# sp-uhh/audio-visual-vad

Measured on AMD Instinct MI355X. Metric: AV frame-pairs/sec (fwd+bwd), higher is better.
Workload: dtype f32; 1 GPU; AV_net fused training step (WaveNet-W0 encoder + ResNet-18 trunk + concat + 2xLSTM1024 + FC, masked BCE, backward, RCCL all-reduce, fused Adam): BASELINE configs[3]/[4] per-GPU shard; per_gpu_frame_pairs=1024, global_frame_pairs=1024, sequences_per_gpu=64, parallelism=dp1, reserved_cus=0, reported_block=median

## Files before the change

### audio-visual-vad_amd/avvad/_lib.py

```python
import ctypes as C
import os

import torch

_HERE = os.path.dirname(os.path.abspath(__file__))
LIB_PATH = os.environ.get("AVVAD_LIB") or os.path.join(os.path.dirname(_HERE), "lib", "libavvad_hip.so")

TRUNK_NCONV = 20
ABI_VERSION = 3
SCORE_CHUNK = 4096
_ERR = {-1: "AVVAD_EINVAL (bad descriptor / unsupported shape)", -2: "AVVAD_EWORKSPACE (workspace too small)",
        -3: "AVVAD_ELAUNCH (kernel launch failed)"}

FP = C.c_void_p


class AvvadError(RuntimeError):
    pass


class GemmDesc(C.Structure):
    _fields_ = [(n, C.c_int) for n in ("M", "N", "K", "lda", "ldb", "ldc", "transA", "transB", "accumulate",
                                       "split_k", "relu_a", "relu_b")]

# ... 13 lines not shown
    _fields_ = [("N", C.c_int), ("H", C.c_int), ("W", C.c_int), ("training", C.c_int), ("momentum", C.c_float),
                ("eps", C.c_float), ("save_for_backward", C.c_int)]


class TrunkParams(C.Structure):
    _fields_ = [("conv_w", FP * TRUNK_NCONV), ("bn_w", FP * TRUNK_NCONV), ("bn_b", FP * TRUNK_NCONV),
                ("bn_rm", FP * TRUNK_NCONV), ("bn_rv", FP * TRUNK_NCONV)]


class TrunkGrads(C.Structure):
    _fields_ = [("conv_w", FP * TRUNK_NCONV), ("bn_w", FP * TRUNK_NCONV), ("bn_b", FP * TRUNK_NCONV)]


class ConvDesc(C.Structure):
    _fields_ = [(n, C.c_int) for n in ("N", "H", "W", "C", "Co", "KS", "stride", "pad")]


class McbDesc(C.Structure):
    _fields_ = [("rows", C.c_int), ("A", C.c_int), ("V", C.c_int), ("D", C.c_int), ("eps", C.c_float),
                ("training", C.c_int), ("momentum", C.c_float), ("save_for_backward", C.c_int)]


class StftDesc(C.Structure):
    _fields_ = [("B", C.c_int), ("L", C.c_long), ("n_fft", C.c_int), ("hop", C.c_int), ("T", C.c_int), ("eps", C.c_float)]


class StftStreamDesc(C.Structure):
    _fields_ = [("B", C.c_int), ("L", C.c_int), ("n_fft", C.c_int), ("hop", C.c_int), ("T", C.c_int), ("M", C.c_int),
                ("eps", C.c_float), ("norm_eps", C.c_float)]

# ... 25 lines not shown
    "avvad_version": (C.c_char_p, []),
    "avvad_abi_version": (C.c_int, []),
    "avvad_set_option": (C.c_int, [C.c_char_p, C.c_int]),
    "avvad_get_option": (C.c_int, [C.c_char_p]),
    "avvad_engine_workspace": (C.c_size_t, []),
    "avvad_gemm_f32": (C.c_int, [FP, FP, FP, FP, C.POINTER(GemmDesc), FP, C.c_size_t, FP]),
    "avvad_wavenet_workspace": (C.c_size_t, [C.POINTER(WavenetDesc)]),
    "avvad_wavenet_fwd": (C.c_int, [FP, C.POINTER(WavenetPtrs), FP, C.POINTER(WavenetDesc), FP, C.c_size_t, FP]),
    "avvad_wavenet_bwd": (C.c_int, [FP, C.POINTER(WavenetPtrs), FP, C.POINTER(WavenetPtrs), FP,
                                    C.POINTER(WavenetDesc), FP, C.c_size_t, FP]),
    "avvad_wavenet_block_fwd": (C.c_int, [FP, FP, FP, FP, FP, FP, C.c_int, C.c_int, C.c_int, FP]),
    "avvad_conv2d_pack_weights": (C.c_int, [FP, FP, FP, C.POINTER(ConvDesc), FP]),
    "avvad_conv2d_fwd": (C.c_int, [FP, FP, FP, C.POINTER(ConvDesc), FP, C.c_size_t, FP]),
    "avvad_conv2d_dgrad": (C.c_int, [FP, FP, FP, C.POINTER(ConvDesc), C.c_int, FP, C.c_size_t, FP]),
    "avvad_conv2d_wgrad": (C.c_int, [FP, FP, FP, C.POINTER(ConvDesc), FP, C.c_size_t, FP]),
    "avvad_conv2d_pack_weights_bf16": (C.c_int, [FP, FP, FP, C.POINTER(ConvDesc), FP]),
    "avvad_conv2d_fwd_bf16": (C.c_int, [FP, FP, FP, C.POINTER(ConvDesc), FP, C.c_size_t, FP]),
    "avvad_conv2d_dgrad_bf16": (C.c_int, [FP, FP, FP, C.POINTER(ConvDesc), C.c_int, FP, C.c_size_t, FP]),
    "avvad_conv2d_wgrad_bf16": (C.c_int, [FP, FP, FP, C.POINTER(ConvDesc), FP, C.c_size_t, FP]),
    "avvad_trunk_workspace": (C.c_size_t, [C.POINTER(TrunkDesc)]),
    "avvad_trunk_activation": (C.c_int, [C.POINTER(TrunkDesc), C.c_int, C.POINTER(C.c_size_t), C.POINTER(C.c_int), C.POINTER(C.c_int),
                                         C.POINTER(C.c_int)]),
    "avvad_trunk_fwd": (C.c_int, [FP, C.POINTER(TrunkParams), FP, C.POINTER(TrunkDesc), FP, C.c_size_t, FP]),
    "avvad_trunk_bwd": (C.c_int, [FP, C.POINTER(TrunkParams), FP, C.POINTER(TrunkGrads), C.POINTER(TrunkDesc), FP,
                                  C.c_size_t, FP]),
    "avvad_lstm_workspace": (C.c_size_t, [C.POINTER(LstmDesc)]),
    "avvad_lstm_layer_fwd": (C.c_int, [FP, FP, FP, FP, FP, FP, C.POINTER(LstmDesc), FP, C.c_size_t, FP]),
    "avvad_lstm_layer_bwd": (C.c_int, [FP, FP, FP, FP, FP, FP, FP, FP, FP, FP, C.POINTER(LstmDesc), FP, C.c_size_t, FP]),
    "avvad_lstm_state_workspace": (C.c_size_t, [C.POINTER(LstmDesc)]),
    "avvad_lstm_layer_fwd_state": (C.c_int, [FP] * 10 + [C.POINTER(LstmDesc), FP, C.c_size_t, FP]),
# ... 107 lines not shown
```

### audio-visual-vad_amd/csrc/bn_kernels.h

```cpp
#pragma once
#include "common.h"

constexpr int BN_MAXC = 1024;
constexpr int MAXC = BN_MAXC;
constexpr int STAT_CHUNKS = 512;

template <int MODE>
__global__ void __launch_bounds__(256)
    col_reduce(const float* __restrict__ x, const float* __restrict__ dy, const float* __restrict__ ymask,
               const float* __restrict__ mean, const float* __restrict__ invstd, long M, int C, long rows_per_chunk,
               double* __restrict__ part, const float* __restrict__ msc = nullptr, const float* __restrict__ msh = nullptr,
               const unsigned char* __restrict__ qmask = nullptr) {
  __shared__ double sm[256 * 8];
  const int t = threadIdx.x;
  const int Q = C >> 2, RL = 256 / Q;
  const int q = t % Q, rl = t / Q;
  double s[4] = {0, 0, 0, 0}, ss[4] = {0, 0, 0, 0};
  float mu[4] = {0, 0, 0, 0}, is[4] = {1, 1, 1, 1};
  float ksc[4] = {0, 0, 0, 0}, ksh[4] = {0, 0, 0, 0};
  if (MODE == 1) {
#pragma unroll
    for (int j = 0; j < 4; ++j) { mu[j] = mean[q * 4 + j]; is[j] = invstd[q * 4 + j]; }
    if (msc) {
#pragma unroll
// ... 158 lines not shown
    const float4 v = reinterpret_cast<const float4*>(x)[i];
    float o[4] = {bn_affine(v.x, sc.x, sh.x), bn_affine(v.y, sc.y, sh.y), bn_affine(v.z, sc.z, sh.z), bn_affine(v.w, sc.w, sh.w)};
    if (idn) {
      const float4 d = IB ? load_quad_bf16(idn, i) : reinterpret_cast<const float4*>(idn)[i];
      if (iscale) {
        o[0] += bn_affine(d.x, a.x, b.x); o[1] += bn_affine(d.y, a.y, b.y);
        o[2] += bn_affine(d.z, a.z, b.z); o[3] += bn_affine(d.w, a.w, b.w);
      } else { o[0] += d.x; o[1] += d.y; o[2] += d.z; o[3] += d.w; }
    }
    if (relu) { o[0] = fmaxf(o[0], 0.f); o[1] = fmaxf(o[1], 0.f); o[2] = fmaxf(o[2], 0.f); o[3] = fmaxf(o[3], 0.f); }
    if constexpr (OB) store_quad_bf16(y, i, o);
    else reinterpret_cast<float4*>(y)[i] = make_float4(o[0], o[1], o[2], o[3]);
    if (qmask_out)
      qmask_out[i] = (unsigned char)((o[0] > 0.f ? 1 : 0) | (o[1] > 0.f ? 2 : 0) | (o[2] > 0.f ? 4 : 0) | (o[3] > 0.f ? 8 : 0));
  }
}

template <bool OB = false>
__global__ void __launch_bounds__(256)
    bn_bwd_apply(const float* __restrict__ x, const float* dy, const float* __restrict__ ymask,
                 const float* __restrict__ mean, const float* __restrict__ invstd, const float* __restrict__ coef,
                 float* dx, float* gout, long nquad, int C, const float* __restrict__ msc = nullptr,
                 const float* __restrict__ msh = nullptr, const unsigned char* __restrict__ qmask = nullptr) {
  const bool fixed = (256 % (C >> 2)) == 0;
  long i = (long)blockIdx.x * blockDim.x + threadIdx.x;
  int c = (int)((i * 4) % C);
  float4 mu = ld4(mean, c), is = ld4(invstd, c), k0 = ld4(coef, c), k1 = ld4(coef + MAXC, c), k2 = ld4(coef + 2 * MAXC, c);
  float4 ms = make_float4(0, 0, 0, 0), mh = ms;
  if (msc) { ms = ld4(msc, c); mh = ld4(msh, c); }
  for (; i < nquad; i += (long)gridDim.x * blockDim.x) {
// ... 16 lines not shown
      if (!(qm & 1u)) g[0] = 0.f;
      if (!(qm & 2u)) g[1] = 0.f;
      if (!(qm & 4u)) g[2] = 0.f;
      if (!(qm & 8u)) g[3] = 0.f;
    } else if (msc) {
      if (!(fmaf(xv.x, ms.x, mh.x) > 0.f)) g[0] = 0.f;
      if (!(fmaf(xv.y, ms.y, mh.y) > 0.f)) g[1] = 0.f;
      if (!(fmaf(xv.z, ms.z, mh.z) > 0.f)) g[2] = 0.f;
      if (!(fmaf(xv.w, ms.w, mh.w) > 0.f)) g[3] = 0.f;
    }
    const float xs[4] = {xv.x, xv.y, xv.z, xv.w};
    const float m4[4] = {mu.x, mu.y, mu.z, mu.w}, i4[4] = {is.x, is.y, is.z, is.w};
    const float a4[4] = {k0.x, k0.y, k0.z, k0.w}, b4[4] = {k1.x, k1.y, k1.z, k1.w}, c4[4] = {k2.x, k2.y, k2.z, k2.w};
    float o[4];
#pragma unroll
    for (int j = 0; j < 4; ++j) {
      const float xh = (xs[j] - m4[j]) * i4[j];
      o[j] = a4[j] * (g[j] - b4[j] - xh * c4[j]);
    }
    if constexpr (OB) store_quad_bf16(dx, i, o);
    else reinterpret_cast<float4*>(dx)[i] = make_float4(o[0], o[1], o[2], o[3]);
    if (gout) reinterpret_cast<float4*>(gout)[i] = make_float4(g[0], g[1], g[2], g[3]);
  }
}
```

### audio-visual-vad_amd/csrc/common.h

```cpp
#pragma once
#include <hip/hip_runtime.h>
#include <stdint.h>
#include <atomic>

#include "avvad.h"

typedef float f32x16 __attribute__((ext_vector_type(16)));
typedef float f32x4 __attribute__((ext_vector_type(4)));

#include <stdio.h>
#define AVVAD_LAUNCH_CHECK()                                                                      \
  do {                                                                                            \
    hipError_t e_ = hipGetLastError();                                                            \
    if (e_ != hipSuccess) {                                                                       \
      fprintf(stderr, "avvad: HIP error '%s' after launch at %s:%d\n", hipGetErrorString(e_), __FILE__, __LINE__); \
      return AVVAD_ELAUNCH;                                                                       \
    }                                                                                             \
  } while (0)

#define AVVAD_ENTER() (void)hipGetLastError()

struct AvvadTune {
  int igemm_variant;
  int no_streamk;
// ... 6 lines not shown
  int wn_no_tail_pair;
  int wn_no_fused_wgrad;
  int no_fixup1;
  int no_buf;
  int wn_flat;
  int wn_dx;
  int wn_grid;
  int wn_bwd_t;
  int bf16;
  int stagger;
  int cls_cap;
  int no_cls;
  int no_fused_stats;
  int no_s2_cls;
  int no_conv64;
  int bwd_max_cus;
  int max_cus;
};
AvvadTune& avvad_tune();
struct BwdCuCap {
  int saved;
  BwdCuCap() : saved(avvad_tune().max_cus) {
    const int b = avvad_tune().bwd_max_cus;
    if (b > 0 && (saved <= 0 || b < saved)) avvad_tune().max_cus = b;
  }
  ~BwdCuCap() { avvad_tune().max_cus = saved; }
};

template <auto Kernel>
int allow_large_lds(size_t bytes, size_t limit) {
// ... 79 lines not shown
```

### audio-visual-vad_amd/csrc/conv64.h

```cpp
#pragma once
#include "common.h"

namespace conv64 {

constexpr int NW = 8;
constexpr int WROWS = 9 * 64;

template <bool FLIP>
__global__ void __launch_bounds__(NW * 64, 2)
    kernel(const float* __restrict__ x, const float* __restrict__ wpk, float* __restrict__ y, const int M, const int H, const int W,
           const unsigned mg_hw, const unsigned mg_w, const int accumulate, double* __restrict__ stat) {
  __shared__ __attribute__((aligned(16))) float wl[WROWS * 64 + NW * 64 * 4];
  const int t = threadIdx.x, lane = t & 63, wave = t >> 6;
  const int li = lane & 31, lh = lane >> 5;
  const __amdgpu_buffer_rsrc_t rx = brsrc2g(x);
  const __amdgpu_buffer_rsrc_t ry = brsrc2g(y);
  const long T = ((long)M + 31) / 32, G = gridDim.x;
  const long t_lo = blockIdx.x * T / G, t_hi = (blockIdx.x + 1) * T / G;
  const int HW = H * W;
  const float* const bl = wl + lh * 256 + li;

  int mbase = 0, rmask = 0, cmask = 0;
  auto tile_ctx = [&](long tile) {
    const int m = (int)tile * 32 + li;
// ... 263 lines not shown
    if (lh == 0) {
      red[(wave * 64 + li) * 2 + 0] = ds0; red[(wave * 64 + li) * 2 + 1] = dq0;
      red[(wave * 64 + li + 32) * 2 + 0] = ds1; red[(wave * 64 + li + 32) * 2 + 1] = dq1;
    }
    __syncthreads();
    if (t < 64) {
      double sa = 0, sb = 0;
#pragma unroll
      for (int w = 0; w < NW; ++w) { sa += red[(w * 64 + t) * 2 + 0]; sb += red[(w * 64 + t) * 2 + 1]; }
      stat[((long)blockIdx.x * 2 + 0) * 64 + t] = sa;
      stat[((long)blockIdx.x * 2 + 1) * 64 + t] = sb;
    }
  }
}

constexpr int WG_WAVES = 12;
constexpr int WG_MAXW = 18;
constexpr int WG_PART = WROWS * 64;

__global__ void __launch_bounds__(WG_WAVES * 64, 3)
    wgrad_kernel(const float* __restrict__ x, const float* __restrict__ dy, float* __restrict__ part, const int NR, const int H,
                 const int W, const unsigned mg_H) {
  constexpr int XP = (WG_MAXW + 2) * 64;
  constexpr int DP = (WG_MAXW + 2) * 64;
  __shared__ __attribute__((aligned(16))) float lds[2 * (3 * XP + DP)];
  const int t = threadIdx.x, lane = t & 63, wave = t >> 6;
  const int li = lane & 31, lh = lane >> 5;
  const int q = wave / 3, kh = wave - q * 3, cb = q >> 1, nb = q & 1;
  for (int i = t; i < 2 * (3 * XP + DP) / 4; i += WG_WAVES * 64) reinterpret_cast<float4*>(lds)[i] = make_float4(0.f, 0.f, 0.f, 0.f);
  const __amdgpu_buffer_rsrc_t rx = brsrc2g(x);
  const __amdgpu_buffer_rsrc_t rd = brsrc2g(dy);
  const long G = gridDim.x;
  const int r_lo = (int)(blockIdx.x * (long)NR / G), r_hi = (int)((blockIdx.x + 1) * (long)NR / G);
  const int per_row = W * 16, items = 4 * per_row;
  int sel[2], goff[2], loff[2];
#pragma unroll
  for (int u = 0; u < 2; ++u) {
    const int idx = t + u * WG_WAVES * 64;
    const int rs = idx / per_row, rem = idx - rs * per_row, px = rem >> 4, c4 = rem & 15;
    sel[u] = idx < items ? rs : -1;
    goff[u] = ((rs < 3 ? rs - 1 : 0) * W + px) * 256 + c4 * 16;
    loff[u] = rs < 3 ? rs * XP + (px + 1) * 64 + c4 * 4 : 3 * XP + px * 64 + c4 * 4;
  }
  f4v st[2];
  auto fetch = [&](int r) {
    const int n = mg_H ? (int)__umulhi((unsigned)r, mg_H) : r, h = r - n * H;
    const int rb = r * W * 256;
#pragma unroll
    for (int u = 0; u < 2; ++u) {
      const bool ok = sel[u] == 3 || (sel[u] >= 0 && (unsigned)(h + sel[u] - 1) < (unsigned)H);
      const int vo = ok ? rb + goff[u] : BUF_OOB;
      st[u] = sel[u] == 3 ? bload4(rd, vo, 0) : bload4(rx, vo, 0);
    }
  };
  auto put = [&](int buf) {
#pragma unroll
    for (int u = 0; u < 2; ++u)
      if (sel[u] >= 0) *reinterpret_cast<f4v*>(lds + buf * (3 * XP + DP) + loff[u]) = st[u];
  };
  f32x16 acc[3];
#pragma unroll
  for (int k = 0; k < 3; ++k)
#pragma unroll
    for (int r = 0; r < 16; ++r) acc[k][r] = 0.f;
  const int nks = (W + 1) >> 1;
  __syncthreads();
  if (r_lo < r_hi) {
    fetch(r_lo);
    put(0);
  }
  __syncthreads();
  for (int r = r_lo; r < r_hi; ++r) {
    const int buf = (r - r_lo) & 1;
    if (r + 1 < r_hi) fetch(r + 1);
    const float* const ap = lds + buf * (3 * XP + DP) + kh * XP + lh * 64 + cb * 32 + li;
    const float* const bp = lds + buf * (3 * XP + DP) + 3 * XP + lh * 64 + nb * 32 + li;
#pragma unroll 3
    for (int ks = 0; ks < nks; ++ks) {
      const float b = bp[ks * 128];
      const float a0 = ap[ks * 128], a1 = ap[ks * 128 + 64], a2 = ap[ks * 128 + 128];
      acc[0] = mfma32(a0, b, acc[0]);
      acc[1] = mfma32(a1, b, acc[1]);
      acc[2] = mfma32(a2, b, acc[2]);
    }
    if (r + 1 < r_hi) put(buf ^ 1);
    __syncthreads();
  }
  float* const P = part + (long)blockIdx.x * WG_PART;
#pragma unroll
  for (int kw = 0; kw < 3; ++kw)
#pragma unroll
    for (int r = 0; r < 16; ++r)
      P[((kh * 3 + kw) * 64 + cb * 32 + mfma32_row(r, lh)) * 64 + nb * 32 + li] = acc[kw][r];
}

__global__ void __launch_bounds__(256)
    wgrad_reduce(const float* __restrict__ part, const int G, float* __restrict__ out) {
  __shared__ float4 red[3][64];
  const int c = threadIdx.x & 63, gq = threadIdx.x >> 6;
  const long e4 = (long)blockIdx.x * 64 + c;
// ... 24 lines not shown
```

### audio-visual-vad_amd/csrc/misc.hip

```cpp
#include "common.h"

extern "C" const char* avvad_version(void) { return "avvad-hip 0.1 (gfx950, fp32 MFMA)"; }
extern "C" int avvad_abi_version(void) { return AVVAD_ABI_VERSION; }

#include <stdlib.h>
#include <string.h>
namespace {
struct OptName { const char* name; const char* env; int AvvadTune::*field; };
const OptName kOpts[] = {
    {"igemm_variant", "AVVAD_IGEMM_VARIANT", &AvvadTune::igemm_variant},
    {"no_streamk", "AVVAD_NO_STREAMK", &AvvadTune::no_streamk},
    {"kmajor", "AVVAD_KMAJOR", &AvvadTune::kmajor},
    {"lstm_no_fused_step", "AVVAD_LSTM_NO_FUSED_STEP", &AvvadTune::lstm_no_fused_step},
    {"lstm_no_persistent", "AVVAD_LSTM_NO_PERSISTENT", &AvvadTune::lstm_no_persistent},
    {"no_stem_kernel", "AVVAD_NO_STEM_KERNEL", &AvvadTune::no_stem_kernel},
    {"no_tall", "AVVAD_NO_TALL", &AvvadTune::no_tall},
    {"wn_no_fused_tail", "AVVAD_WN_NO_FUSED_TAIL", &AvvadTune::wn_no_fused_tail},
    {"wn_no_tail_pair", "AVVAD_WN_NO_TAIL_PAIR", &AvvadTune::wn_no_tail_pair},
    {"wn_no_fused_wgrad", "AVVAD_WN_NO_FUSED_WGRAD", &AvvadTune::wn_no_fused_wgrad},
    {"wn_bwd_t", "AVVAD_WN_BWD_T", &AvvadTune::wn_bwd_t},
    {"no_buf", "AVVAD_NO_BUF", &AvvadTune::no_buf},
    {"no_fixup1", "AVVAD_NO_FIXUP1", &AvvadTune::no_fixup1},
    {"no_conv64", "AVVAD_NO_CONV64", &AvvadTune::no_conv64},
    {"no_s2_cls", "AVVAD_NO_S2_CLS", &AvvadTune::no_s2_cls},
    {"wn_flat", "AVVAD_WN_FLAT", &AvvadTune::wn_flat},
    {"wn_grid", "AVVAD_WN_GRID", &AvvadTune::wn_grid},
    {"wn_dx", "AVVAD_WN_DX", &AvvadTune::wn_dx},
    {"bf16", "AVVAD_BF16", &AvvadTune::bf16},
    {"no_fused_stats", "AVVAD_NO_FUSED_STATS", &AvvadTune::no_fused_stats},
    {"no_cls", "AVVAD_NO_CLS", &AvvadTune::no_cls},
    {"cls_cap", "AVVAD_CLS_CAP", &AvvadTune::cls_cap},
    {"stagger", "AVVAD_STAGGER", &AvvadTune::stagger},
    {"max_cus", "AVVAD_MAX_CUS", &AvvadTune::max_cus},
    {"bwd_max_cus", "AVVAD_BWD_MAX_CUS", &AvvadTune::bwd_max_cus},
};
int parse_opt(const char* name, const char* v) {
  if (!strcmp(name, "igemm_variant")) return v[0] == 'd' ? 0 : (v[0] == 's' ? 1 : (v[0] == 'w' ? 2 : atoi(v)));
  if (!strcmp(name, "no_streamk")) return v[0] == 'a' ? 1 : (v[0] >= '0' && v[0] <= '9' && !v[1] ? 10 + (v[0] - '0') : atoi(v));
  if (!strcmp(name, "max_cus") || !strcmp(name, "bwd_max_cus") || !strcmp(name, "wn_flat") || !strcmp(name, "wn_grid") || !strcmp(name, "wn_dx") || !strcmp(name, "wn_bwd_t") || !strcmp(name, "no_fixup1") || !strcmp(name, "cls_cap")) return atoi(v);
  return (v[0] && strcmp(v, "0")) ? 1 : 0;
}
}

AvvadTune& avvad_tune() {
  static AvvadTune t = [] {
    AvvadTune x;
    memset(&x, 0, sizeof(x));
    x.igemm_variant = -1;
    for (const OptName& o : kOpts) {
      const char* v = getenv(o.env);
      if (v && v[0]) x.*(o.field) = parse_opt(o.name, v);
    }
    return x;
  }();
// ... 279 lines not shown
```

### audio-visual-vad_amd/csrc/trunk.hip

```cpp
#include "bgemm.h"
#include "conv64.h"

using convop::Geom;

namespace {

#include "bn_kernels.h"

constexpr int NCONV = AVVAD_TRUNK_NCONV;

struct ConvSpec {
  int cin, cout, ks, stride, pad;
  int stage;
  int role;
};

struct Plan {
  int N, H, W;
  int h[6], w[6];
  ConvSpec conv[NCONV];
  Geom geom[NCONV];
  size_t wf[NCONV], wd[NCONV];
  size_t wf16[NCONV], wd16[NCONV];
  size_t bn_scale, bn_shift, bn_mean, bn_invstd;
// ... 706 lines not shown
}
static inline igemm::TapSched tap_sched(const Geom& g, int tiles_per_tap) {
  const int NP = cdiv(g.N, 128) * 128;
  const int lsh = ((g.Ho - 1) * g.stride - g.pad + 2 > g.H - 1) ? 1 : 0, lsw = ((g.Wo - 1) * g.stride - g.pad + 2 > g.W - 1) ? 1 : 0;
  return igemm::TapSched{g.Ho, g.Wo, tiles_per_tap, NP / 32, 3, 1, lsh, 1, lsw};
}
static int conv_wgrad_tap(const float* x, const float* dy, float* pk, const Geom& g, hipStream_t s, float* slab) {
  const int M = 9 * g.C;
  const igemm::TapSched sc = tap_sched(g, (g.C / 128) * cdiv(g.Co, 128));
  convop::WgradXTap a{x, g, M, g.C, g.N, convop::div_magic(g.C), sc};
  convop::ColDyTap b{dy, g, g.Co, g.C, g.N, sc};
  igemm::EpiTap e{pk, g.Co, nullptr, 0};
  e.Mrows = M; e.sched = sc;
  return igemm::launch_cls(a, b, e, M, g.Co, s, slab);
}
static int conv64_wgrad(const float* x, const float* dy, float* pk, const Geom& g, hipStream_t s, float* slab) {
  const int NR = g.N * g.H;
  const int grid = NR < conv64_cus() ? NR : conv64_cus();
  hipLaunchKernelGGL(conv64::wgrad_kernel, dim3(grid), dim3(conv64::WG_WAVES * 64), 0, s, x, dy, slab, NR, g.H, g.W,
                     convop::div_magic((unsigned)g.H));
  hipLaunchKernelGGL(conv64::wgrad_reduce, dim3(conv64::WG_PART / 256), dim3(256), 0, s, (const float*)slab, grid, pk);
  AVVAD_LAUNCH_CHECK();
  return AVVAD_OK;
}
static int conv_wgrad(const float* x, const float* dy, float* pk, const Geom& g, hipStream_t s, float* slab) {
  const ConvForm f = wgrad_form(g, false, slab);
  switch (f.form) {
    case STEM: {
      const int LDW = (g.W + 6) | 1;
      const int nb = g.N < 256 ? g.N : 256;
      hipLaunchKernelGGL(stem_wgrad_mfma, dim3(nb), dim3(256), (size_t)(g.H + 6) * LDW * sizeof(float), s, x, dy, slab, g.N, g.H, g.W,
                         g.Ho, g.Wo, LDW);
      hipLaunchKernelGGL(stem_wgrad_reduce, dim3(49 * 64 / 32), dim3(256), 0, s, slab, nb, pk);
      AVVAD_LAUNCH_CHECK();
      return AVVAD_OK;
    }
    case CONV64: return conv64_wgrad(x, dy, pk, g, s, slab);
    case TAP: return conv_wgrad_tap(x, dy, pk, g, s, slab);
    default: return f.buf ? conv_wgrad_t<true>(x, dy, pk, g, f, s, slab) : conv_wgrad_t<false>(x, dy, pk, g, f, s, slab);
  }
}

static int conv_fwd16(const float* x16, const float* wf16, float* y, const Geom& g, hipStream_t s, float* slab, double* stat) {
  if (!bf16_conv_ok(g)) return AVVAD_EINVAL;
  const ConvForm f = fwd_form(g, true, slab);
  if (f.form == CONV64) return conv64_launch(true, false, x16, wf16, y, g, 0, s, stat);
  Geom gp = g;
  gp.C = g.C / 2;
  if (f.form == CLS) {
    const int MB = cdiv(g.N, 128), P = g.Ho * g.Wo;
    const igemm::ClassSched sc = fwd_sched(g, 64);
    const igemm::ClassRow cr{P, convop::div_magic(P)};
// ... 93 lines not shown
  const int C = p->conv[i].cout;
  StatCtx sc = stat_ctx(p, ws, M, C);
  if (const int n = fused_chunks(p, i, d)) {
    sc.nchunk = n;
  } else if (d->training) {
    hipLaunchKernelGGL(col_reduce<0>, dim3(sc.nchunk), dim3(256), 0, s, craw, (const float*)nullptr, (const float*)nullptr,
                       (const float*)nullptr, (const float*)nullptr, M, C, sc.rows_per_chunk, sc.part);
  }
  hipLaunchKernelGGL(bn_finalize, dim3(cdiv(C, FIN_CH)), dim3(256), 0, s, sc.part, sc.nchunk, M, C, prm->bn_w[i], prm->bn_b[i],
                     prm->bn_rm[i], prm->bn_rv[i], d->training, d->momentum, d->eps, ws + p->bn_scale + i * MAXC,
                     ws + p->bn_shift + i * MAXC, ws + p->bn_mean + i * MAXC, ws + p->bn_invstd + i * MAXC);
  AVVAD_LAUNCH_CHECK();
  return AVVAD_OK;
}

static int bn_backward(Plan* p, float* ws, int i, const float* xraw, const float* dy, const float* ymask, float* dx,
                       float* gout, long M, const avvad_trunk_params* prm, const avvad_trunk_grads* g,
                       const avvad_trunk_desc* d, hipStream_t s, bool own_relu = false, const unsigned char* qmask = nullptr,
                       bool out16 = false, int reduced_chunks = 0) {
  const int C = p->conv[i].cout;
  StatCtx sc = stat_ctx(p, ws, M, C);
  const float* mean = ws + p->bn_mean + i * MAXC;
  const float* invstd = ws + p->bn_invstd + i * MAXC;
  const float* msc = own_relu ? ws + p->bn_scale + i * MAXC : (const float*)nullptr;
  const float* msh = own_relu ? ws + p->bn_shift + i * MAXC : (const float*)nullptr;
  if (own_relu) ymask = nullptr;
  const bool qred = out16 && qmask != nullptr;
  if (reduced_chunks > 0)
    sc.nchunk = reduced_chunks;
  else
    hipLaunchKernelGGL(col_reduce<1>, dim3(sc.nchunk), dim3(256), 0, s, xraw, dy, qred ? (const float*)nullptr : ymask, mean, invstd, M, C,
                       sc.rows_per_chunk, sc.part, msc, msh, qred ? qmask : (const unsigned char*)nullptr);
  hipLaunchKernelGGL(bn_bwd_finalize, dim3(cdiv(C, FIN_CH)), dim3(256), 0, s, sc.part, sc.nchunk, M, C, prm->bn_w[i], invstd,
                     d->training, g->bn_w[i], g->bn_b[i], ws + p->coef);
  const long nq = M * C / 4;
  auto apply = out16 ? bn_bwd_apply<true> : bn_bwd_apply<false>;
  hipLaunchKernelGGL(apply, dim3(ew_grid(nq)), dim3(256), 0, s, xraw, dy, qmask ? (const float*)nullptr : ymask, mean, invstd,
                     ws + p->coef, dx, gout, nq, C, msc, msh, qmask);
  AVVAD_LAUNCH_CHECK();
  return AVVAD_OK;
}

}

static bool conv_geom(const avvad_conv_desc* d, Geom* g) {
  if (!d || d->N <= 0 || d->H <= 0 || d->W <= 0 || d->C <= 0 || d->Co <= 0 || d->KS <= 0 || d->stride <= 0 || d->pad < 0)
    return false;
  const int Ho = (d->H + 2 * d->pad - d->KS) / d->stride + 1, Wo = (d->W + 2 * d->pad - d->KS) / d->stride + 1;
  if (Ho <= 0 || Wo <= 0 || (d->stride != 1 && d->stride != 2)) return false;
// ... 40 lines not shown
#endif
extern "C" int avvad_conv2d_dgrad(const float* dy, const float* wd, float* dx, const avvad_conv_desc* d, int accumulate,
                                  void* ws, size_t ws_bytes, avvad_stream_t s) {
  AVVAD_ENTER();
  Geom g;
  if (!dy || !wd || !dx || !conv_geom(d, &g) || ws_misaligned(ws)) return AVVAD_EINVAL;
  return conv_dgrad(dy, wd, dx, g, accumulate, (hipStream_t)s, slab_of(ws, ws_bytes));
}
extern "C" int avvad_conv2d_wgrad(const float* x, const float* dy, float* dw_packed, const avvad_conv_desc* d, void* ws,
                                  size_t ws_bytes, avvad_stream_t s) {
  AVVAD_ENTER();
  Geom g;
  if (!x || !dy || !dw_packed || !conv_geom(d, &g) || ws_misaligned(ws)) return AVVAD_EINVAL;
  return conv_wgrad(x, dy, dw_packed, g, (hipStream_t)s, slab_of(ws, ws_bytes));
}

namespace {
__global__ void pack_weights_bf16(const float* __restrict__ w, __bf16* __restrict__ wf16, __bf16* __restrict__ wd16, int Co, int C, int KS) {
  const int T = KS * KS, n = Co * C * T;
  for (int i = blockIdx.x * blockDim.x + threadIdx.x; i < n; i += gridDim.x * blockDim.x) {
    int r = i;
    const int tap = r % T; r /= T;
    const int c = r % C; const int co = r / C;
    const __bf16 v = (__bf16)w[i];
    wf16[(long)co * (T * C) + ((c >> 6) * T + tap) * 64 + (c & 63)] = v;
    if (wd16) wd16[(long)c * (T * Co) + ((co >> 6) * T + tap) * 64 + (co & 63)] = v;
  }
}
}
extern "C" int avvad_conv2d_pack_weights_bf16(const float* w_oihw, void* wf16, void* wd16, const avvad_conv_desc* d, avvad_stream_t s) {
  AVVAD_ENTER();
// ... 142 lines not shown
  float* G1 = ws + p.G[1];
  float* G2 = ws + p.G[2];
  float* G3 = ws + p.G[3];
  hipLaunchKernelGGL(avgpool_bwd, dim3(ew_grid(N * p.h[5] * p.w[5] * 512)), dim3(256), 0, s, dfeat, G0, d->N,
                     p.h[5] * p.w[5], 512);
  const bool b16 = native_bf16();
  auto wgrad = [&](int i, const float* xin, const float* dyraw) -> int {
    if (!g->conv_w[i]) return AVVAD_OK;
    if (b16 && i > 0) return conv_wgrad16(xin, dyraw, ws + p.wg[i], p.geom[i], s, ws + p.slab);
    return conv_wgrad(xin, dyraw, ws + p.wg[i], p.geom[i], s, ws + p.slab);
  };
  auto dgrad = [&](const float* dyv, int i, float* dxv, int accumulate) -> int {
    if (b16) return conv_dgrad16(dyv, ws + p.wd16[i], dxv, p.geom[i], accumulate, s, ws + p.slab);
    return conv_dgrad(dyv, ws + p.wd[i], dxv, p.geom[i], accumulate, s, ws + p.slab);
  };
  int ci = NCONV;
  for (int st = 3; st >= 0; --st)
    for (int b = 1; b >= 0; --b) {
      const bool ds = (b == 0 && st > 0);
      ci -= ds ? 3 : 2;
      const int i1 = ci, i2 = ci + 1, id = ci + 2;
      const size_t* o = p.blk[st * 2 + b];
      const float* x = (st == 0 && b == 0) ? ws + p.p0 : (b == 1 ? ws + p.blk[st * 2][4] : ws + p.blk[st * 2 - 1][4]);
      const long M = N * p.h[st + 2] * p.w[st + 2];
      const unsigned char* qmb = reinterpret_cast<const unsigned char*>(ws + p.qm[st * 2 + b]);
      if (ds) {
        if ((rc = bn_backward(&p, ws, i2, ws + o[2], G0, ws + o[4], G1, nullptr, M, prm, g, d, s, false, qmb, b16))) return rc;
        if ((rc = bn_backward(&p, ws, id, ws + o[3], G0, ws + o[4], G2, nullptr, M, prm, g, d, s, false, qmb, b16))) return rc;
        if ((rc = wgrad(id, x, G2))) return rc;
        if ((rc = dgrad(G2, id, G3, 0))) return rc;
      } else {
        if ((rc = bn_backward(&p, ws, i2, ws + o[2], G0, ws + o[4], G1, G3, M, prm, g, d, s, false, qmb, b16))) return rc;
      }
      if ((rc = wgrad(i2, ws + o[1], G1))) return rc;
      if ((rc = dgrad(G1, i2, G2, 0))) return rc;
      if ((rc = bn_backward(&p, ws, i1, ws + o[0], G2, ws + o[1], G1, nullptr, M, prm, g, d, s, true, nullptr, b16))) return rc;
      if ((rc = wgrad(i1, x, G1))) return rc;
      if ((rc = dgrad(G1, i1, G3, 1))) return rc;
      float* t = G0; G0 = G3; G3 = t;
    }
  if (g->conv_w[0] || g->bn_w[0] || g->bn_b[0]) {
    float* g0 = ws + p.g0;
    const bool fuse0 = !avvad_tune().no_fused_stats;
    int grid0 = ew_grid(N * p.h[1] * p.w[1] * 16);
    if (fuse0 && grid0 > 2048) grid0 = 2048;
    hipLaunchKernelGGL(stem_pool_relu_bwd, dim3(grid0), dim3(256), 0, s, ws + p.c0,
                       ws + p.bn_scale, ws + p.bn_shift, reinterpret_cast<const unsigned*>(ws + p.am), G0, g0, d->N, p.h[1], p.w[1],
                       p.h[2], p.w[2], fuse0 ? ws + p.bn_mean : (const float*)nullptr, fuse0 ? ws + p.bn_invstd : (const float*)nullptr,
                       fuse0 ? reinterpret_cast<double*>(ws + p.part) : (double*)nullptr);
    const long M0 = N * p.h[1] * p.w[1];
    if ((rc = bn_backward(&p, ws, 0, ws + p.c0, g0, nullptr, g0, nullptr, M0, prm, g, d, s, false, nullptr, false, fuse0 ? grid0 : 0))) return rc;
    if ((rc = wgrad(0, frames, g0))) return rc;
// ... 22 lines not shown
```

### include/avvad.h

```cpp
#ifndef AVVAD_H
#define AVVAD_H

#include <stddef.h>
#include <stdint.h>

#ifdef __cplusplus
extern "C" {
#endif

typedef void* avvad_stream_t;

#define AVVAD_OK 0
#define AVVAD_EINVAL (-1)
#define AVVAD_EWORKSPACE (-2)
#define AVVAD_ELAUNCH (-3)

#define AVVAD_ABI_VERSION 3
const char* avvad_version(void);
int avvad_abi_version(void);

int avvad_set_option(const char* name, int value);
int avvad_get_option(const char* name);

typedef struct {
// ... 80 lines not shown
  float* bn_w[AVVAD_TRUNK_NCONV];
  float* bn_b[AVVAD_TRUNK_NCONV];
} avvad_trunk_grads;

typedef struct {
  int N, H, W, C, Co, KS, stride, pad;
} avvad_conv_desc;
int avvad_conv2d_pack_weights(const float* w_oihw, float* wf, float* wd, const avvad_conv_desc* d,
                              avvad_stream_t s);
int avvad_conv2d_fwd(const float* x, const float* wf, float* y, const avvad_conv_desc* d, void* ws,
                     size_t ws_bytes, avvad_stream_t s);
int avvad_conv2d_dgrad(const float* dy, const float* wd, float* dx, const avvad_conv_desc* d,
                       int accumulate, void* ws, size_t ws_bytes, avvad_stream_t s);
int avvad_conv2d_wgrad(const float* x, const float* dy, float* dw_packed, const avvad_conv_desc* d, void* ws,
                       size_t ws_bytes, avvad_stream_t s);

int avvad_conv2d_pack_weights_bf16(const float* w_oihw, void* wf16, void* wd16, const avvad_conv_desc* d, avvad_stream_t s);
int avvad_conv2d_fwd_bf16(const void* x16, const void* wf16, float* y, const avvad_conv_desc* d, void* ws, size_t ws_bytes,
                          avvad_stream_t s);
int avvad_conv2d_dgrad_bf16(const void* dy16, const void* wd16, float* dx, const avvad_conv_desc* d, int accumulate,
                            void* ws, size_t ws_bytes, avvad_stream_t s);
int avvad_conv2d_wgrad_bf16(const void* x16, const void* dy16, float* dw_packed, const avvad_conv_desc* d, void* ws,
                            size_t ws_bytes, avvad_stream_t s);

size_t avvad_trunk_workspace(const avvad_trunk_desc* d);
int avvad_trunk_activation(const avvad_trunk_desc* d, int index, size_t* offset_floats, int* C, int* H, int* W);
int avvad_trunk_fwd(const float* frames, const avvad_trunk_params* p, float* feat ,
                    const avvad_trunk_desc* d, void* ws, size_t ws_bytes, avvad_stream_t s);
int avvad_trunk_bwd(const float* frames, const avvad_trunk_params* p, const float* dfeat,
                    const avvad_trunk_grads* g, const avvad_trunk_desc* d, void* ws, size_t ws_bytes,
// ... 204 lines not shown
```

Before: 60830 frame-pairs/s.

## Fuse BN backward apply into conv64 weight-gradient kernel for layer1 blocks

For the stage-0 (64-channel) ResNet blocks in the fp32 path, the BN backward elementwise apply (ReLU mask, normalization gradient, gout write) now runs inside the conv64 wgrad kernel. The kernel applies it to dy tiles as they are loaded into LDS and writes dc/gout out along the way. This drops a separate full-tensor apply pass and one re-read of dy and dc for those layers. In exchange the wgrad kernel carries extra register and LDS pressure and extra global stores. It also adds a public API entry point and an env toggle to disable the fusion.

```diff
diff --git a/audio-visual-vad_amd/avvad/_lib.py b/audio-visual-vad_amd/avvad/_lib.py
--- a/audio-visual-vad_amd/avvad/_lib.py
+++ b/audio-visual-vad_amd/avvad/_lib.py
@@ -51,6 +51,10 @@
 
 class ConvDesc(C.Structure):
     _fields_ = [(n, C.c_int) for n in ("N", "H", "W", "C", "Co", "KS", "stride", "pad")]
+
+
+class BnBwdDesc(C.Structure):
+    _fields_ = [(n, FP) for n in ("xraw", "mean", "invstd", "msc", "msh", "qmask")]
 
 
 class McbDesc(C.Structure):
@@ -106,6 +110,7 @@
     "avvad_conv2d_fwd": (C.c_int, [FP, FP, FP, C.POINTER(ConvDesc), FP, C.c_size_t, FP]),
     "avvad_conv2d_dgrad": (C.c_int, [FP, FP, FP, C.POINTER(ConvDesc), C.c_int, FP, C.c_size_t, FP]),
     "avvad_conv2d_wgrad": (C.c_int, [FP, FP, FP, C.POINTER(ConvDesc), FP, C.c_size_t, FP]),
+    "avvad_conv2d_wgrad_bn": (C.c_int, [FP, FP, C.POINTER(BnBwdDesc), FP, FP, FP, FP, C.POINTER(ConvDesc), C.c_int, FP, C.c_size_t, FP]),
     "avvad_conv2d_pack_weights_bf16": (C.c_int, [FP, FP, FP, C.POINTER(ConvDesc), FP]),
     "avvad_conv2d_fwd_bf16": (C.c_int, [FP, FP, FP, C.POINTER(ConvDesc), FP, C.c_size_t, FP]),
     "avvad_conv2d_dgrad_bf16": (C.c_int, [FP, FP, FP, C.POINTER(ConvDesc), C.c_int, FP, C.c_size_t, FP]),
diff --git a/audio-visual-vad_amd/csrc/bn_kernels.h b/audio-visual-vad_amd/csrc/bn_kernels.h
--- a/audio-visual-vad_amd/csrc/bn_kernels.h
+++ b/audio-visual-vad_amd/csrc/bn_kernels.h
@@ -196,6 +196,11 @@
     if (qmask_out)
       qmask_out[i] = (unsigned char)((o[0] > 0.f ? 1 : 0) | (o[1] > 0.f ? 2 : 0) | (o[2] > 0.f ? 4 : 0) | (o[3] > 0.f ? 8 : 0));
   }
+}
+
+__device__ __forceinline__ float bn_bwd_elem(float x, float g, float mu, float is, float k0, float k1, float k2) {
+  const float xh = (x - mu) * is;
+  return k0 * (g - k1 - xh * k2);
 }
 
 template <bool OB = false>
@@ -242,10 +247,7 @@
     const float a4[4] = {k0.x, k0.y, k0.z, k0.w}, b4[4] = {k1.x, k1.y, k1.z, k1.w}, c4[4] = {k2.x, k2.y, k2.z, k2.w};
     float o[4];
 #pragma unroll
-    for (int j = 0; j < 4; ++j) {
-      const float xh = (xs[j] - m4[j]) * i4[j];
-      o[j] = a4[j] * (g[j] - b4[j] - xh * c4[j]);
-    }
+    for (int j = 0; j < 4; ++j) o[j] = bn_bwd_elem(xs[j], g[j], m4[j], i4[j], a4[j], b4[j], c4[j]);
     if constexpr (OB) store_quad_bf16(dx, i, o);
     else reinterpret_cast<float4*>(dx)[i] = make_float4(o[0], o[1], o[2], o[3]);
     if (gout) reinterpret_cast<float4*>(gout)[i] = make_float4(g[0], g[1], g[2], g[3]);
diff --git a/audio-visual-vad_amd/csrc/common.h b/audio-visual-vad_amd/csrc/common.h
--- a/audio-visual-vad_amd/csrc/common.h
+++ b/audio-visual-vad_amd/csrc/common.h
@@ -44,6 +44,7 @@
   int no_fused_stats;
   int no_s2_cls;
   int no_conv64;
+  int no_l1_bn_fuse;
   int bwd_max_cus;
   int max_cus;
 };
diff --git a/audio-visual-vad_amd/csrc/conv64.h b/audio-visual-vad_amd/csrc/conv64.h
--- a/audio-visual-vad_amd/csrc/conv64.h
+++ b/audio-visual-vad_amd/csrc/conv64.h
@@ -301,13 +301,25 @@
   }
 }
 
+struct BnApply {
+  const float* xraw;
+  const float* mean;
+  const float* invstd;
+  const float* coef;
+  const float* msc;
+  const float* msh;
+  const unsigned char* qmask;
+  float* dc;
+  float* gout;
+};
 constexpr int WG_WAVES = 12;
 constexpr int WG_MAXW = 18;
 constexpr int WG_PART = WROWS * 64;
 
+template <bool BN>
 __global__ void __launch_bounds__(WG_WAVES * 64, 3)
     wgrad_kernel(const float* __restrict__ x, const float* __restrict__ dy, float* __restrict__ part, const int NR, const int H,
-                 const int W, const unsigned mg_H) {
+                 const int W, const unsigned mg_H, const BnApply bn) {
   constexpr int XP = (WG_MAXW + 2) * 64;
   constexpr int DP = (WG_MAXW + 2) * 64;
   __shared__ __attribute__((aligned(16))) float lds[2 * (3 * XP + DP)];
@@ -330,6 +342,21 @@
     loff[u] = rs < 3 ? rs * XP + (px + 1) * 64 + c4 * 4 : 3 * XP + px * 64 + c4 * 4;
   }
   f4v st[2];
+  const int du = sel[0] == 3 ? 0 : (sel[1] == 3 ? 1 : -1);
+  auto dgo = [&]() -> int { return du == 0 ? goff[0] : goff[1]; };
+  const __amdgpu_buffer_rsrc_t rbx = brsrc2g(bn.xraw);
+  const __amdgpu_buffer_rsrc_t rdc = brsrc2g(bn.dc);
+  const __amdgpu_buffer_rsrc_t rgo = brsrc2g(bn.gout);
+  __shared__ __attribute__((aligned(16))) float cf[BN ? 7 * 64 : 4];
+  if (BN && t < 7 * 16) {
+    const int row = t >> 4, c = (t & 15) * 4;
+    const float* const src = row == 0 ? bn.mean : row == 1 ? bn.invstd : row < 5 ? bn.coef + (row - 2) * MAXC
+                           : bn.qmask != nullptr ? nullptr : (row == 5 ? bn.msc : bn.msh);
+    const f4v z = {0.f, 0.f, 0.f, 0.f};
+    *reinterpret_cast<f4v*>(cf + row * 64 + c) = src != nullptr ? *reinterpret_cast<const f4v*>(src + c) : z;
+  }
+  f4v bxr = {0.f, 0.f, 0.f, 0.f};
+  unsigned bqm = 0;
   auto fetch = [&](int r) {
     const int n = mg_H ? (int)__umulhi((unsigned)r, mg_H) : r, h = r - n * H;
     const int rb = r * W * 256;
@@ -339,8 +366,28 @@
       const int vo = ok ? rb + goff[u] : BUF_OOB;
       st[u] = sel[u] == 3 ? bload4(rd, vo, 0) : bload4(rx, vo, 0);
     }
-  };
-  auto put = [&](int buf) {
+    if (BN) {
+      const int bvo = du >= 0 ? rb + dgo() : BUF_OOB;
+      bxr = bload4(rbx, bvo, 0);
+      if (bn.qmask != nullptr && du >= 0) bqm = bn.qmask[bvo >> 4];
+    }
+  };
+  auto put = [&](int buf, int r) {
+    if (BN && du >= 0) {
+      const int bvo = r * W * 256 + dgo();
+      const float* const cfq = cf + ((dgo() & 255) >> 2);
+      f4v g = du == 0 ? st[0] : st[1], dc;
+#pragma unroll
+      for (int j = 0; j < 4; ++j) {
+        const bool pass = bn.qmask != nullptr ? ((bqm >> j) & 1u) != 0 : fmaf(bxr[j], cfq[320 + j], cfq[384 + j]) > 0.f;
+        if (!pass) g[j] = 0.f;
+        dc[j] = bn_bwd_elem(bxr[j], g[j], cfq[j], cfq[64 + j], cfq[128 + j], cfq[192 + j], cfq[256 + j]);
+        __builtin_amdgcn_sched_barrier(0);
+      }
+      bstore4(dc, rdc, bvo, 0);
+      if (bn.gout != nullptr) bstore4(g, rgo, bvo, 0);
+      if (du == 0) st[0] = dc; else st[1] = dc;
+    }
 #pragma unroll
     for (int u = 0; u < 2; ++u)
       if (sel[u] >= 0) *reinterpret_cast<f4v*>(lds + buf * (3 * XP + DP) + loff[u]) = st[u];
@@ -354,7 +401,7 @@
   __syncthreads();
   if (r_lo < r_hi) {
     fetch(r_lo);
-    put(0);
+    put(0, r_lo);
   }
   __syncthreads();
   for (int r = r_lo; r < r_hi; ++r) {
@@ -370,7 +417,7 @@
       acc[1] = mfma32(a1, b, acc[1]);
       acc[2] = mfma32(a2, b, acc[2]);
     }
-    if (r + 1 < r_hi) put(buf ^ 1);
+    if (r + 1 < r_hi) put(buf ^ 1, r + 1);
     __syncthreads();
   }
   float* const P = part + (long)blockIdx.x * WG_PART;
diff --git a/audio-visual-vad_amd/csrc/misc.hip b/audio-visual-vad_amd/csrc/misc.hip
--- a/audio-visual-vad_amd/csrc/misc.hip
+++ b/audio-visual-vad_amd/csrc/misc.hip
@@ -28,6 +28,7 @@
     {"wn_dx", "AVVAD_WN_DX", &AvvadTune::wn_dx},
     {"bf16", "AVVAD_BF16", &AvvadTune::bf16},
     {"no_fused_stats", "AVVAD_NO_FUSED_STATS", &AvvadTune::no_fused_stats},
+    {"no_l1_bn_fuse", "AVVAD_NO_L1_BN_FUSE", &AvvadTune::no_l1_bn_fuse},
     {"no_cls", "AVVAD_NO_CLS", &AvvadTune::no_cls},
     {"cls_cap", "AVVAD_CLS_CAP", &AvvadTune::cls_cap},
     {"stagger", "AVVAD_STAGGER", &AvvadTune::stagger},
@@ -37,7 +38,7 @@
 int parse_opt(const char* name, const char* v) {
   if (!strcmp(name, "igemm_variant")) return v[0] == 'd' ? 0 : (v[0] == 's' ? 1 : (v[0] == 'w' ? 2 : atoi(v)));
   if (!strcmp(name, "no_streamk")) return v[0] == 'a' ? 1 : (v[0] >= '0' && v[0] <= '9' && !v[1] ? 10 + (v[0] - '0') : atoi(v));
-  if (!strcmp(name, "max_cus") || !strcmp(name, "bwd_max_cus") || !strcmp(name, "wn_flat") || !strcmp(name, "wn_grid") || !strcmp(name, "wn_dx") || !strcmp(name, "wn_bwd_t") || !strcmp(name, "no_fixup1") || !strcmp(name, "cls_cap")) return atoi(v);
+  if (!strcmp(name, "max_cus") || !strcmp(name, "bwd_max_cus") || !strcmp(name, "wn_flat") || !strcmp(name, "wn_grid") || !strcmp(name, "wn_dx") || !strcmp(name, "wn_bwd_t") || !strcmp(name, "no_fixup1") || !strcmp(name, "cls_cap") || !strcmp(name, "no_l1_bn_fuse")) return atoi(v);
   return (v[0] && strcmp(v, "0")) ? 1 : 0;
 }
 }
diff --git a/audio-visual-vad_amd/csrc/trunk.hip b/audio-visual-vad_amd/csrc/trunk.hip
--- a/audio-visual-vad_amd/csrc/trunk.hip
+++ b/audio-visual-vad_amd/csrc/trunk.hip
@@ -1,11 +1,11 @@
 #include "bgemm.h"
+
+using convop::Geom;
+
+namespace {
+
+#include "bn_kernels.h"
 #include "conv64.h"
-
-using convop::Geom;
-
-namespace {
-
-#include "bn_kernels.h"
 
 constexpr int NCONV = AVVAD_TRUNK_NCONV;
 
@@ -744,17 +744,24 @@
   e.Mrows = M; e.sched = sc;
   return igemm::launch_cls(a, b, e, M, g.Co, s, slab);
 }
-static int conv64_wgrad(const float* x, const float* dy, float* pk, const Geom& g, hipStream_t s, float* slab) {
+static int conv64_wgrad(const float* x, const float* dy, float* pk, const Geom& g, hipStream_t s, float* slab,
+                        const conv64::BnApply* bn = nullptr) {
   const int NR = g.N * g.H;
   const int grid = NR < conv64_cus() ? NR : conv64_cus();
-  hipLaunchKernelGGL(conv64::wgrad_kernel, dim3(grid), dim3(conv64::WG_WAVES * 64), 0, s, x, dy, slab, NR, g.H, g.W,
-                     convop::div_magic((unsigned)g.H));
+  if (bn)
+    hipLaunchKernelGGL(conv64::wgrad_kernel<true>, dim3(grid), dim3(conv64::WG_WAVES * 64), 0, s, x, dy, slab, NR, g.H, g.W,
+                       convop::div_magic((unsigned)g.H), *bn);
+  else
+    hipLaunchKernelGGL(conv64::wgrad_kernel<false>, dim3(grid), dim3(conv64::WG_WAVES * 64), 0, s, x, dy, slab, NR, g.H, g.W,
+                       convop::div_magic((unsigned)g.H), conv64::BnApply{});
   hipLaunchKernelGGL(conv64::wgrad_reduce, dim3(conv64::WG_PART / 256), dim3(256), 0, s, (const float*)slab, grid, pk);
   AVVAD_LAUNCH_CHECK();
   return AVVAD_OK;
 }
-static int conv_wgrad(const float* x, const float* dy, float* pk, const Geom& g, hipStream_t s, float* slab) {
+static int conv_wgrad(const float* x, const float* dy, float* pk, const Geom& g, hipStream_t s, float* slab,
+                      const conv64::BnApply* bn = nullptr) {
   const ConvForm f = wgrad_form(g, false, slab);
+  if (bn && f.form != CONV64) return AVVAD_EINVAL;
   switch (f.form) {
     case STEM: {
       const int LDW = (g.W + 6) | 1;
@@ -765,7 +772,7 @@
       AVVAD_LAUNCH_CHECK();
       return AVVAD_OK;
     }
-    case CONV64: return conv64_wgrad(x, dy, pk, g, s, slab);
+    case CONV64: return conv64_wgrad(x, dy, pk, g, s, slab, bn);
     case TAP: return conv_wgrad_tap(x, dy, pk, g, s, slab);
     default: return f.buf ? conv_wgrad_t<true>(x, dy, pk, g, f, s, slab) : conv_wgrad_t<false>(x, dy, pk, g, f, s, slab);
   }
@@ -889,25 +896,37 @@
   return AVVAD_OK;
 }
 
+static int bn_bwd_sums(Plan* p, float* ws, int i, const float* xraw, const float* dy, const float* ymask, long M, hipStream_t s,
+                       bool own_relu, const unsigned char* qmask, bool out16) {
+  const int C = p->conv[i].cout;
+  const StatCtx sc = stat_ctx(p, ws, M, C);
+  const float* msc = own_relu ? ws + p->bn_scale + i * MAXC : (const float*)nullptr;
+  const float* msh = own_relu ? ws + p->bn_shift + i * MAXC : (const float*)nullptr;
+  if (own_relu) ymask = nullptr;
+  const bool qred = out16 && qmask != nullptr;
+  hipLaunchKernelGGL(col_reduce<1>, dim3(sc.nchunk), dim3(256), 0, s, xraw, dy, qred ? (const float*)nullptr : ymask,
+                     ws + p->bn_mean + i * MAXC, ws + p->bn_invstd + i * MAXC, M, C, sc.rows_per_chunk, sc.part, msc, msh,
+                     qred ? qmask : (const unsigned char*)nullptr);
+  return sc.nchunk;
+}
+static void bn_bwd_fin(Plan* p, float* ws, int i, int nchunk, long M, const avvad_trunk_params* prm, const avvad_trunk_grads* g,
+                       const avvad_trunk_desc* d, hipStream_t s) {
+  const int C = p->conv[i].cout;
+  hipLaunchKernelGGL(bn_bwd_finalize, dim3(cdiv(C, FIN_CH)), dim3(256), 0, s, reinterpret_cast<const double*>(ws + p->part), nchunk, M, C,
+                     prm->bn_w[i], ws + p->bn_invstd + i * MAXC, d->training, g->bn_w[i], g->bn_b[i], ws + p->coef);
+}
 static int bn_backward(Plan* p, float* ws, int i, const float* xraw, const float* dy, const float* ymask, float* dx,
                        float* gout, long M, const avvad_trunk_params* prm, const avvad_trunk_grads* g,
                        const avvad_trunk_desc* d, hipStream_t s, bool own_relu = false, const unsigned char* qmask = nullptr,
                        bool out16 = false, int reduced_chunks = 0) {
   const int C = p->conv[i].cout;
-  StatCtx sc = stat_ctx(p, ws, M, C);
   const float* mean = ws + p->bn_mean + i * MAXC;
   const float* invstd = ws + p->bn_invstd + i * MAXC;
   const float* msc = own_relu ? ws + p->bn_scale + i * MAXC : (const float*)nullptr;
   const float* msh = own_relu ? ws + p->bn_shift + i * MAXC : (const float*)nullptr;
+  const int nchunk = reduced_chunks > 0 ? reduced_chunks : bn_bwd_sums(p, ws, i, xraw, dy, ymask, M, s, own_relu, qmask, out16);
+  bn_bwd_fin(p, ws, i, nchunk, M, prm, g, d, s);
   if (own_relu) ymask = nullptr;
-  const bool qred = out16 && qmask != nullptr;
-  if (reduced_chunks > 0)
-    sc.nchunk = reduced_chunks;
-  else
-    hipLaunchKernelGGL(col_reduce<1>, dim3(sc.nchunk), dim3(256), 0, s, xraw, dy, qred ? (const float*)nullptr : ymask, mean, invstd, M, C,
-                       sc.rows_per_chunk, sc.part, msc, msh, qred ? qmask : (const unsigned char*)nullptr);
-  hipLaunchKernelGGL(bn_bwd_finalize, dim3(cdiv(C, FIN_CH)), dim3(256), 0, s, sc.part, sc.nchunk, M, C, prm->bn_w[i], invstd,
-                     d->training, g->bn_w[i], g->bn_b[i], ws + p->coef);
   const long nq = M * C / 4;
   auto apply = out16 ? bn_bwd_apply<true> : bn_bwd_apply<false>;
   hipLaunchKernelGGL(apply, dim3(ew_grid(nq)), dim3(256), 0, s, xraw, dy, qmask ? (const float*)nullptr : ymask, mean, invstd,
@@ -978,7 +997,28 @@
   if (!x || !dy || !dw_packed || !conv_geom(d, &g) || ws_misaligned(ws)) return AVVAD_EINVAL;
   return conv_wgrad(x, dy, dw_packed, g, (hipStream_t)s, slab_of(ws, ws_bytes));
 }
-
+static bool bn_desc_ok(const avvad_bn_bwd_desc* bn) {
+  return bn && bn->xraw && bn->mean && bn->invstd && (bn->qmask || (bn->msc && bn->msh));
+}
+extern "C" int avvad_conv2d_wgrad_bn(const float* x, const float* dy, const avvad_bn_bwd_desc* bn, const float* coef, float* dc,
+                                     float* gout, float* dw_packed, const avvad_conv_desc* d, int fused, void* ws, size_t ws_bytes,
+                                     avvad_stream_t s) {
+  AVVAD_ENTER();
+  Geom g;
+  if (!x || !dy || !bn_desc_ok(bn) || !coef || !dc || !dw_packed || !conv_geom(d, &g) || ws_misaligned(ws)) return AVVAD_EINVAL;
+  float* slab = slab_of(ws, ws_bytes);
+  if (wgrad_form(g, false, slab).form != CONV64) return AVVAD_EINVAL;
+  const float* msc = bn->qmask ? (const float*)nullptr : bn->msc;
+  const float* msh = bn->qmask ? (const float*)nullptr : bn->msh;
+  if (fused) {
+    const conv64::BnApply a{bn->xraw, bn->mean, bn->invstd, coef, msc, msh, bn->qmask, dc, gout};
+    return conv_wgrad(x, dy, dw_packed, g, (hipStream_t)s, slab, &a);
+  }
+  const long nq = (long)g.N * g.H * g.W * 16;
+  hipLaunchKernelGGL(bn_bwd_apply<false>, dim3(ew_grid(nq)), dim3(256), 0, (hipStream_t)s, bn->xraw, dy, (const float*)nullptr, bn->mean,
+                     bn->invstd, coef, dc, gout, nq, 64, msc, msh, bn->qmask);
+  return conv_wgrad(x, dc, dw_packed, g, (hipStream_t)s, slab);
+}
 namespace {
 __global__ void pack_weights_bf16(const float* __restrict__ w, __bf16* __restrict__ wf16, __bf16* __restrict__ wd16, int Co, int C, int KS) {
   const int T = KS * KS, n = Co * C * T;
@@ -1151,6 +1191,20 @@
     if (b16) return conv_dgrad16(dyv, ws + p.wd16[i], dxv, p.geom[i], accumulate, s, ws + p.slab);
     return conv_dgrad(dyv, ws + p.wd[i], dxv, p.geom[i], accumulate, s, ws + p.slab);
   };
+  const bool l1_fuse = !b16 && !(avvad_tune().no_l1_bn_fuse & 1);
+  auto l1_apply = [&](int st, int i) {
+    return st == 0 && l1_fuse && g->conv_w[i] && wgrad_form(p.geom[i], false, true).form == CONV64;
+  };
+  auto bn_wgrad = [&](int i, const float* xin, const float* xraw, const float* dyv, const float* ymask, float* dc, float* gout, long M,
+                      bool own_relu, const unsigned char* qmask) -> int {
+    const int chunks = bn_bwd_sums(&p, ws, i, xraw, dyv, ymask, M, s, own_relu, qmask, false);
+    bn_bwd_fin(&p, ws, i, chunks, M, prm, g, d, s);
+    const conv64::BnApply a{xraw, ws + p.bn_mean + i * MAXC, ws + p.bn_invstd + i * MAXC, ws + p.coef,
+                            own_relu ? ws + p.bn_scale + i * MAXC : (const float*)nullptr,
+                            own_relu ? ws + p.bn_shift + i * MAXC : (const float*)nullptr, own_relu ? (const unsigned char*)nullptr : qmask,
+                            dc, gout};
+    return conv_wgrad(xin, dyv, ws + p.wg[i], p.geom[i], s, ws + p.slab, &a);
+  };
   int ci = NCONV;
   for (int st = 3; st >= 0; --st)
     for (int b = 1; b >= 0; --b) {
@@ -1167,12 +1221,21 @@
         if ((rc = wgrad(id, x, G2))) return rc;
         if ((rc = dgrad(G2, id, G3, 0))) return rc;
       } else {
-        if ((rc = bn_backward(&p, ws, i2, ws + o[2], G0, ws + o[4], G1, G3, M, prm, g, d, s, false, qmb, b16))) return rc;
+        if (l1_apply(st, i2)) {
+          if ((rc = bn_wgrad(i2, ws + o[1], ws + o[2], G0, ws + o[4], G1, G3, M, false, qmb))) return rc;
+        } else {
+          if ((rc = bn_backward(&p, ws, i2, ws + o[2], G0, ws + o[4], G1, G3, M, prm, g, d, s, false, qmb, b16))) return rc;
+          if ((rc = wgrad(i2, ws + o[1], G1))) return rc;
+        }
       }
-      if ((rc = wgrad(i2, ws + o[1], G1))) return rc;
+      if (ds && (rc = wgrad(i2, ws + o[1], G1))) return rc;
       if ((rc = dgrad(G1, i2, G2, 0))) return rc;
-      if ((rc = bn_backward(&p, ws, i1, ws + o[0], G2, ws + o[1], G1, nullptr, M, prm, g, d, s, true, nullptr, b16))) return rc;
-      if ((rc = wgrad(i1, x, G1))) return rc;
+      if (l1_apply(st, i1)) {
+        if ((rc = bn_wgrad(i1, x, ws + o[0], G2, nullptr, G1, nullptr, M, true, nullptr))) return rc;
+      } else {
+        if ((rc = bn_backward(&p, ws, i1, ws + o[0], G2, ws + o[1], G1, nullptr, M, prm, g, d, s, true, nullptr, b16))) return rc;
+        if ((rc = wgrad(i1, x, G1))) return rc;
+      }
       if ((rc = dgrad(G1, i1, G3, 1))) return rc;
       float* t = G0; G0 = G3; G3 = t;
     }
diff --git a/include/avvad.h b/include/avvad.h
--- a/include/avvad.h
+++ b/include/avvad.h
@@ -118,6 +118,18 @@
                        int accumulate, void* ws, size_t ws_bytes, avvad_stream_t s);
 int avvad_conv2d_wgrad(const float* x, const float* dy, float* dw_packed, const avvad_conv_desc* d, void* ws,
                        size_t ws_bytes, avvad_stream_t s);
+
+typedef struct {
+  const float* xraw;
+  const float* mean;
+  const float* invstd;
+  const float* msc;
+  const float* msh;
+  const unsigned char* qmask;
+} avvad_bn_bwd_desc;
+int avvad_conv2d_wgrad_bn(const float* x, const float* dy, const avvad_bn_bwd_desc* bn, const float* coef, float* dc,
+                          float* gout, float* dw_packed, const avvad_conv_desc* d, int fused, void* ws, size_t ws_bytes,
+                          avvad_stream_t s);
 
 int avvad_conv2d_pack_weights_bf16(const float* w_oihw, void* wf16, void* wd16, const avvad_conv_desc* d, avvad_stream_t s);
 int avvad_conv2d_fwd_bf16(const void* x16, const void* wf16, float* y, const avvad_conv_desc* d, void* ws, size_t ws_bytes,
```

After: 61220 frame-pairs/s, median of 6. No clear change (+0.7%).
